# HKUST-Aerial-Robotics/A-LOAM

Hardware: AMD Instinct MI355X
Metric: HDL-64 scans/sec (whole node) (higher is better)
Workload: dtype f32 features / f64 solve

## Files before the change

### a-loam_amd/csrc/odometry_kernels.hip

```cpp
#include "aloam_device.hpp"
#include "aloam_trig.hpp"
#include "lm_device.hpp"
#include "odometry_solve_device.hpp"
#include "odometry_kernels.hpp"

namespace aloam {

#define ALOAM_PHASE(name) asm volatile("; ##PHASE " name)
#ifdef ALOAM_PHASE_CLOCK
__device__ unsigned long long g_phase_clock_odo[2][32];
#define ALOAM_BG_CLOCK(slot) do { if (threadIdx.x == 0 && blockIdx.x == 1) { atomicAdd(&g_phase_clock_odo[0][slot], (unsigned long long)__builtin_readcyclecounter()); atomicAdd(&g_phase_clock_odo[1][slot], 1ull); } } while (0)
#else
#define ALOAM_BG_CLOCK(slot) do { } while (0)
#endif
#ifdef ALOAM_ASSOC_STATS
__device__ unsigned long long g_assoc_stats[2][32];
#define ALOAM_STAT(cls, i, v) do { if ((threadIdx.x & 63) == 0) atomicAdd(&g_assoc_stats[cls][i], (unsigned long long)(v)); } while (0)
#else
#define ALOAM_STAT(cls, i, v) do { } while (0)
#endif

__device__ __forceinline__ float4 transform_to_start(const float4& p, const OdomState& st) {
  double q[4] = {st.para_q[0], st.para_q[1], st.para_q[2], st.para_q[3]};
  if (q[3] < 0.0) { q[0] = -q[0]; q[1] = -q[1]; q[2] = -q[2]; q[3] = -q[3]; }
  double o[3];
  quat_rotate(q, (double)p.x, (double)p.y, (double)p.z, o);
  return make_float4((float)(o[0] + st.para_t[0]), (float)(o[1] + st.para_t[1]), (float)(o[2] + st.para_t[2]), p.w);
}

constexpr float kCell3Surf = 0.5f;
constexpr float kCell3Corner = 0.75f;
constexpr float kCell3CoarseFactor = 4.0f, kCell2 = 2.625f;
constexpr unsigned kIdxMask = (1u << 20) - 1u;
__device__ __forceinline__ float cell3_of(int which) { return which == 0 ? kCell3Corner : kCell3Surf; }

__device__ __forceinline__ unsigned hash3(int a, int b, int c) {
  return ((unsigned)a * 73856093u) ^ ((unsigned)b * 19349663u) ^ ((unsigned)c * 83492791u);
}

constexpr int kFusedMaxN = 65535, kFusedMaxH = 16384;
constexpr int kWalkKeys = kMaxRings + 8;

__device__ __forceinline__ void walk_tables(const float4* __restrict__ pts, int n, int R, int* __restrict__ walk, int* s_walk, int* s_flag, int tid) {
  const int S = R + 8, lane = tid & 63;
  int* s_first = s_walk;
  int* s_last = s_walk + kWalkKeys;
  for (int k = tid; k < kWalkKeys; k += 1024) { s_first[k] = 0x7fffffff; s_last[k] = -1; }
  __syncthreads();
  for (int base = 0; base < n; base += 1024) {
    const int i = base + tid;
    const int key = i < n ? (int)pts[i].w : -1;
    const int prev = __shfl_up(key, 1, 64), next = __shfl_down(key, 1, 64);
    if (key >= 0 && key < S) {
      if (lane == 0 || prev != key) atomicMin(&s_first[key], i);
      if (lane == 63 || next != key) atomicMax(&s_last[key], i);
    }
  }
  __syncthreads();
  if (tid == 0) {
    int run = n;
    for (int k = S - 1; k >= 0; --k) { run = min(run, s_first[k]); s_first[k] = run; walk[k] = run; }
    run = -1;
    for (int k = 0; k < S; ++k) { run = max(run, s_last[k]); s_last[k] = run; walk[S + k] = run; }
    bool nearly = true;
    for (int k = 3; k < S; ++k) nearly = nearly && s_last[k - 3] < s_first[k];
    s_flag[1] = nearly ? 1 : 2;
  }
  __syncthreads();
}
__host__ __device__ __forceinline__ bool fused_takes(int n, int H) { return n <= kFusedMaxN && H <= kFusedMaxH; }

template <bool NEXT>
struct BuildSrc {
  int n, set;
  const float4* pts;
  __device__ __forceinline__ BuildSrc(const OdomArgs& a, const SeqMeta& m, int b, int which) {
    set = NEXT ? m.parity : m.parity ^ 1;
    n = which == 0 ? (NEXT ? m.n_less_sharp : m.n_corner_last) : (NEXT ? m.n_less_flat : m.n_surf_last);
    pts = which == 0 ? row_of(a.less_sharp, set, b, (long long)a.R * kLessSharpPerRing) : row_of(a.less_flat, set, b, (long long)a.cap);
  }
};

template <bool NEXT>
__device__ __forceinline__ void build_grids_fused(const OdomArgs& a, int b, int which) {
  constexpr int U = 4;
  const int tid = threadIdx.x, lane = tid & 63, wave = tid >> 6;
  if (seq_idle(a.active, b, NEXT ? kSeqActive : kSeqSolve)) return;
  const SeqMeta m = a.meta[b];
  const BuildSrc<NEXT> src(a, m, b, which);
  const int n = src.n;
  const float4* pts = src.pts;
  const GridView g = grid_view(a, b, which, src.set);
  const int H = g.H;
  if (!fused_takes(n, H)) return;
  extern __shared__ __attribute__((aligned(16))) int lds[];
  unsigned* tab = reinterpret_cast<unsigned*>(lds);
  int* s_part = lds + 3 * (H / 2);
  int* s_flag = s_part + 48;
  int* s_walk = s_flag + 8;
  int* const starts[3] = {g.start3, g.start3c, g.start2};
  if (n == 0) {
    for (int t = 0; t < 3; ++t) for (int h = tid; h <= H; h += 1024) starts[t][h] = 0;
    if (tid < 3) g.flags[tid] = 0;
    return;
  }
  ALOAM_BG_CLOCK(0);
  for (int w = tid; w < 3 * (H / 2); w += 1024) tab[w] = 0u;
  if (tid < 2) s_flag[tid] = 0;
  __syncthreads();
  ALOAM_BG_CLOCK(1);
  const float inv0 = 1.0f / cell3_of(which), inv1 = 1.0f / (cell3_of(which) * kCell3CoarseFactor), inv2 = 1.0f / kCell2;
  const unsigned hm = (unsigned)(H - 1);
  auto buckets = [&](const float4& p, int key, unsigned* h) {
    h[0] = hash3((int)floorf(p.x * inv0), (int)floorf(p.y * inv0), (int)floorf(p.z * inv0)) & hm;
    h[1] = hash3((int)floorf(p.x * inv1), (int)floorf(p.y * inv1), (int)floorf(p.z * inv1)) & hm;
    h[2] = hash3((int)floorf(p.x * inv2), (int)floorf(p.y * inv2), key) & hm;
  };
  auto fetch = [&](int base, float4* p) {
#pragma unroll
    for (int u = 0; u < U; ++u) { const int i = base + u * 1024 + tid; p[u] = pts[i < n ? i : n - 1]; }
  };
  {
    int bad = 0, unsorted = 0;
    for (int base = 0; base < n; base += U * 1024) {
      float4 p[U];
      float pw[U];
      fetch(base, p);
#pragma unroll
      for (int u = 0; u < U; ++u) { const int i = base + u * 1024 + tid; pw[u] = pts[i < n ? (i > 0 ? i - 1 : 0) : n - 1].w; }
#pragma unroll
      for (int u = 0; u < U; ++u) {
        if (base + u * 1024 + tid >= n) continue;
        const int key = (int)p[u].w;
        if (key < 0 || key > a.R || !(fabsf(p[u].x) < 4096.f && fabsf(p[u].y) < 4096.f && fabsf(p[u].z) < 4096.f)) bad = 1;
        if (key < (int)pw[u]) unsorted = 1;
        unsigned h[3];
        buckets(p[u], key, h);
#pragma unroll
        for (int t = 0; t < 3; ++t) atomicAdd(&tab[t * (H / 2) + (h[t] >> 1)], 1u << ((h[t] & 1u) * 16));
      }
    }
    if (bad) atomicOr(&s_flag[0], 1);
    if (unsorted) atomicOr(&s_flag[1], 1);
  }
  __syncthreads();
  ALOAM_BG_CLOCK(2);
  if (s_flag[1] && !s_flag[0]) walk_tables(pts, n, a.R, g.walk, s_walk, s_flag, tid);
  if (tid < 3) g.flags[tid] = tid == 2 ? 0 : s_flag[tid];
  ALOAM_BG_CLOCK(3);
  {
    const int wpt = H / 2048;
    int local[3], inc[3];
#pragma unroll
    for (int t = 0; t < 3; ++t) {
      local[t] = 0;
      for (int k = 0; k < wpt; ++k) { const unsigned w = tab[t * (H / 2) + tid * wpt + k]; local[t] += (int)(w & 0xffffu) + (int)(w >> 16); }
      inc[t] = wave_scan_i32<false>(local[t]);
      if (lane == 63) s_part[t * 16 + wave] = inc[t];
    }
    __syncthreads();
#pragma unroll
    for (int t = 0; t < 3; ++t) {
      int run = inc[t] - local[t];
#pragma unroll 1
      for (int w = 0; w < wave; ++w) run += s_part[t * 16 + w];
      int* st = starts[t] + tid * wpt * 2;
      for (int k = 0; k < wpt; ++k) {
        const unsigned w = tab[t * (H / 2) + tid * wpt + k];
        const int c0 = (int)(w & 0xffffu), c1 = (int)(w >> 16);
        st[2 * k] = run; st[2 * k + 1] = run + c0;
        tab[t * (H / 2) + tid * wpt + k] = (unsigned)run | ((unsigned)(run + c0) << 16);
        run += c0 + c1;
      }
      if (tid == 1023) starts[t][H] = run;
    }
  }
  __syncthreads();
  ALOAM_BG_CLOCK(4);
  for (int base = 0; base < n; base += U * 1024) {
    float4 p[U];
    fetch(base, p);
#pragma unroll
    for (int u = 0; u < U; ++u) {
      const int i = base + u * 1024 + tid;
      if (i >= n) continue;
      const int key = (int)p[u].w;
      unsigned h[3];
      buckets(p[u], key, h);
      unsigned pos[3];
#pragma unroll
      for (int t = 0; t < 3; ++t) {
        const unsigned sh = (h[t] & 1u) * 16;
        pos[t] = (atomicAdd(&tab[t * (H / 2) + (h[t] >> 1)], 1u << sh) >> sh) & 0xffffu;
      }
      const float4 e = make_float4(p[u].x, p[u].y, p[u].z, __uint_as_float((unsigned)i | ((unsigned)(key + 1) << 20)));
      g.sorted3[pos[0]] = e;
      g.sorted3c[pos[1]] = e;
      g.sorted2[pos[2]] = e;
    }
  }
  ALOAM_BG_CLOCK(5);
#ifdef ALOAM_PHASE_CLOCK
  __syncthreads();
  ALOAM_BG_CLOCK(6);
#endif
}

__global__ __launch_bounds__(1024) void k_build_grids_fused(OdomArgs a) { build_grids_fused<false>(a, blockIdx.y, blockIdx.x); }
__global__ __launch_bounds__(1024) void k_build_grids_fused_next(OdomArgs a) {
  const int G = gridDim.x;
  for (int r = 0, i = blockIdx.x; i < 2 * a.B; ++r, i += G) {
    build_grids_fused<true>(a, i >> 1, (i ^ r) & 1);
    __syncthreads();
  }
}

constexpr int kBgWaves = 4;
constexpr int kBgUnroll = 4;
template <bool NEXT>
__device__ __forceinline__ void build_grids(const OdomArgs& a) {
  constexpr int U = kBgUnroll;
  const int b = blockIdx.y, which = blockIdx.x / 3, tid = threadIdx.x;
  const int pass_lo = blockIdx.x % 3, pass_hi = pass_lo + 1;
  if (seq_idle(a.active, b, NEXT ? kSeqActive : kSeqSolve)) return;
  const SeqMeta m = a.meta[b];
  const BuildSrc<NEXT> src(a, m, b, which);
  const int n = src.n;
  const float4* pts = src.pts;
  const GridView g = grid_view(a, b, which, src.set);
  if (fused_takes(n, g.H)) return;
  extern __shared__ __attribute__((aligned(16))) int lds[];
  int* cnt = lds;
  int* part = lds + g.H;
  int* s_flag = part + 1024;
  if (tid < 2) s_flag[tid] = n >= (1 << 20) && tid == 0 ? 1 : 0;
  if (n == 0) {
    for (int pass = pass_lo; pass < pass_hi; ++pass) { int* st = pass == 0 ? g.start3 : pass == 1 ? g.start3c : g.start2; for (int h = tid; h <= g.H; h += 1024) st[h] = 0; }
    if (tid < 3 && pass_lo == 0) g.flags[tid] = 0;
    return;
  }
  auto fetch = [&](int base, float4* p) {
#pragma unroll
    for (int u = 0; u < U; ++u) { const int i = base + u * 1024 + tid; p[u] = pts[i < n ? i : n - 1]; }
  };
  for (int pass = pass_lo; pass < pass_hi; ++pass) {
    const bool g3 = pass < 2;
    const float cell = pass == 0 ? cell3_of(which) : pass == 1 ? cell3_of(which) * kCell3CoarseFactor : kCell2;
    const float inv = 1.0f / cell;
    int* start = pass == 0 ? g.start3 : pass == 1 ? g.start3c : g.start2;
    float4* sorted = pass == 0 ? g.sorted3 : pass == 1 ? g.sorted3c : g.sorted2;
    __syncthreads();
    for (int h = tid; h < g.H; h += 1024) cnt[h] = 0;
    __syncthreads();
    float4 p[U], pn[U];
    float pw[U], pwn[U];
    fetch(0, p);
    if (pass == 0) {
#pragma unroll
      for (int u = 0; u < U; ++u) { const int i = u * 1024 + tid; pw[u] = pts[i < n ? (i > 0 ? i - 1 : 0) : n - 1].w; }
    }
    int bad = 0, unsorted = 0;
    for (int base = 0; base < n; base += U * 1024) {
      if (base + U * 1024 < n) {
        fetch(base + U * 1024, pn);
        if (pass == 0) {
#pragma unroll
          for (int u = 0; u < U; ++u) { const int i = base + U * 1024 + u * 1024 + tid; pwn[u] = pts[i < n ? i - 1 : n - 1].w; }
        }
      }
#pragma unroll
      for (int u = 0; u < U; ++u) {
        if (base + u * 1024 + tid >= n) continue;
        const int key = (int)p[u].w;
        if (pass == 0) {
          if (key < 0 || key > a.R || !(fabsf(p[u].x) < 4096.f && fabsf(p[u].y) < 4096.f && fabsf(p[u].z) < 4096.f)) bad = 1;
          if (key < (int)pw[u]) unsorted = 1;
        }
        const int ix = (int)floorf(p[u].x * inv), iy = (int)floorf(p[u].y * inv);
        const int iz = g3 ? (int)floorf(p[u].z * inv) : key;
        atomicAdd(&cnt[hash3(ix, iy, iz) & (g.H - 1)], 1);
      }
#pragma unroll
      for (int u = 0; u < U; ++u) { p[u] = pn[u]; pw[u] = pwn[u]; }
    }
    if (pass == 0) {
      if (bad) atomicOr(&s_flag[0], 1);
      if (unsorted) atomicOr(&s_flag[1], 1);
    }
    __syncthreads();
    if (pass == 0 && tid < 3) g.flags[tid] = tid == 2 ? 0 : (tid == 1 ? 2 * s_flag[1] : s_flag[0]);
    const int per = g.H / 1024;
    int local = 0;
    for (int k = 0; k < per; ++k) local += cnt[tid * per + k];
    int total;
    int run = block_exclusive_scan<int, 1024>(local, part, &total);
    for (int k = 0; k < per; ++k) { const int c = cnt[tid * per + k]; cnt[tid * per + k] = run; start[tid * per + k] = run; run += c; }
    if (tid == 1023) start[g.H] = run;
    __syncthreads();
    fetch(0, p);
    for (int base = 0; base < n; base += U * 1024) {
      if (base + U * 1024 < n) fetch(base + U * 1024, pn);
#pragma unroll
      for (int u = 0; u < U; ++u) {
        const int i = base + u * 1024 + tid;
        if (i >= n) continue;
        const int key = (int)p[u].w;
        const int ix = (int)floorf(p[u].x * inv), iy = (int)floorf(p[u].y * inv);
        const int iz = g3 ? (int)floorf(p[u].z * inv) : key;
        const int pos = atomicAdd(&cnt[hash3(ix, iy, iz) & (g.H - 1)], 1);
        sorted[pos] = make_float4(p[u].x, p[u].y, p[u].z, __uint_as_float((unsigned)i | ((unsigned)(key + 1) << 20)));
      }
#pragma unroll
      for (int u = 0; u < U; ++u) p[u] = pn[u];
    }
  }
}

__global__ __launch_bounds__(1024, kBgWaves) void k_build_grids(OdomArgs a) { build_grids<false>(a); }
__global__ __launch_bounds__(1024, kBgWaves) void k_build_grids_next(OdomArgs a) { build_grids<true>(a); }

__device__ __forceinline__ float walk_dist(const float4& p, const float4& sel) {
  return (p.x - sel.x) * (p.x - sel.x) + (p.y - sel.y) * (p.y - sel.y) + (p.z - sel.z) * (p.z - sel.z);
}

__device__ __forceinline__ unsigned long long wave_min_u64(unsigned long long v) {
  return wave_min_packed(v);
}

__device__ __forceinline__ void ring2d(int r, int t, int* dx, int* dy) {
  const int w = 2 * r + 1;
  if (t < w) { *dx = -r + t; *dy = -r; }
  else if (t < 2 * w) { *dx = -r + (t - w); *dy = r; }
  else { const int u = t - 2 * w, side = u / (w - 2); *dy = -r + 1 + u % (w - 2); *dx = side ? r : -r; }
}
__device__ __forceinline__ void shell3d(int r, int c, int* dx, int* dy, int* dz) {
  const int w = 2 * r + 1, nface = w * w;
  if (c < 2 * nface) { const int f = c / nface, q = c % nface; *dz = f ? r : -r; *dy = q / w - r; *dx = q % w - r; }
  else { const int q = c - 2 * nface; *dz = -r + 1 + q / (8 * r); ring2d(r, q % (8 * r), dx, dy); }
}

template <int kSweep> struct Kept { float4 p[kSweep]; bool a[kSweep]; bool ok; };

template <int kSweep, class F>
__device__ __forceinline__ void wave_sweep(const float4* __restrict__ sorted, int s0, int cnt, int lane, int* row, F&& f, Kept<kSweep>* keep = nullptr) {
  const int incl = wave_scan_i32<false>(cnt);
  const int total = __builtin_amdgcn_readlane(incl, 63);
  const int excl = incl - cnt;
  int carry = 0;
  for (int base = 0; base < total; base += kSweep * 64) {
    const int slot = excl - base;
    const int rows = total - base > (kSweep - 1) * 64 ? kSweep : (total - base + 63) >> 6;
#pragma unroll
    for (int u = 0; u < kSweep; ++u) if (u < rows) row[u * 64 + lane] = 0;
    __builtin_amdgcn_wave_barrier();
    if (cnt > 0 && slot >= 0 && slot < rows * 64) row[slot] = lane + 1;
    __builtin_amdgcn_wave_barrier();
    int own[kSweep];
#pragma unroll
    for (int u = 0; u < kSweep; ++u) own[u] = u < rows ? row[u * 64 + lane] : 0;
    __builtin_amdgcn_wave_barrier();
    float4 p[kSweep];
#pragma unroll
    for (int u = 0; u < kSweep; ++u) {
      p[u] = make_float4(0.f, 0.f, 0.f, 0.f);
      if (u < rows) {
        if (lane == 0 && carry > own[u]) own[u] = carry;
        own[u] = wave_scan_i32<true>(own[u]);
        carry = __builtin_amdgcn_readlane(own[u], 63);
        const int i = base + u * 64 + lane;
        const int os = __shfl(s0, own[u] - 1, 64), oe = __shfl(excl, own[u] - 1, 64);
        const int at = i < total ? os + (i - oe) : 0;
        p[u] = sorted[at];
      }
    }
#pragma unroll
    for (int u = 0; u < kSweep; ++u) {
      const bool act = u < rows && base + u * 64 + lane < total;
      if (keep) { keep->p[u] = p[u]; keep->a[u] = act; }
      if (act) f(p[u]);
    }
  }
  if (keep) keep->ok = total <= kSweep * 64;
}

__device__ __forceinline__ float cell_gap(float s, int c, float cell) {
  const float lo = (float)c * cell, hi = lo + cell;
  const float gap = s < lo ? lo - s : (s > hi ? s - hi : 0.f);
  return gap > 1e-3f ? gap - 1e-3f : 0.f;
}

struct Track { unsigned long long v; float x, y, z; };
__device__ __forceinline__ void track_take(Track& t, bool ok, unsigned long long v, const float4& p) {
  const bool k = ok && v < t.v;
  t.v = k ? v : t.v; t.x = k ? p.x : t.x; t.y = k ? p.y : t.y; t.z = k ? p.z : t.z;
}

template <int kSweep>
__device__ __forceinline__ unsigned long long wave_nn(const GridView& g, bool bad, int which, const float4* pts, int n, const float4& sel, int lane, int* row, Track& mine, Kept<kSweep>& kept) {
  unsigned long long best = ~0ull;
  auto visit = [&](const float4& p) {
    const float ddx = p.x - sel.x, ddy = p.y - sel.y, ddz = p.z - sel.z;
    const float d = (ddx * ddx + ddy * ddy) + ddz * ddz;
    const unsigned wb = __float_as_uint(p.w);
    track_take(mine, true, ((unsigned long long)__float_as_uint(d) << 32) | ((wb & kIdxMask) << 12) | (wb >> 20), p);
  };
  if (!bad) {
    const float cell = cell3_of(which);
    {
      const float inv = 1.0f / cell;
      const int cx = (int)floorf(sel.x * inv), cy = (int)floorf(sel.y * inv), cz = (int)floorf(sel.z * inv);
      int s0 = 0, cnt = 0;
      if (lane < 27) {
        const unsigned h = hash3(cx + lane % 3 - 1, cy + (lane % 9) / 3 - 1, cz + lane / 9 - 1) & (unsigned)(g.H - 1);
        s0 = g.start3[h];
        cnt = g.start3[h + 1] - s0;
      }
      wave_sweep<kSweep>(g.sorted3, s0, cnt, lane, row, visit, &kept);
      best = wave_min_u64(mine.v);
      const float bound = (1.0f - 0.01f) * cell;
      if (best != ~0ull && __uint_as_float((unsigned)(best >> 32)) <= bound * bound) return best;
    }
    const float cellc = cell * kCell3CoarseFactor, invc = 1.0f / cellc;
    const int ux = (int)floorf(sel.x * invc), uy = (int)floorf(sel.y * invc), uz = (int)floorf(sel.z * invc);
    for (int r = 1;; ++r) {
      const int ncell = r == 1 ? 27 : 24 * r * r + 2;
      const float limit = best != ~0ull ? fminf(__uint_as_float((unsigned)(best >> 32)), 25.0f) : 25.0f;
      for (int cb = 0; cb < ncell; cb += 64) {
        const int c = cb + lane;
        int s0 = 0, cnt = 0;
        if (c < ncell) {
          int dx, dy, dz;
          if (r == 1) { dz = c / 9 - 1; dy = (c % 9) / 3 - 1; dx = c % 3 - 1; }
          else shell3d(r, c, &dx, &dy, &dz);
          const float gx = cell_gap(sel.x, ux + dx, cellc), gy = cell_gap(sel.y, uy + dy, cellc), gz = cell_gap(sel.z, uz + dz, cellc);
          if (((gx * gx + gy * gy) + gz * gz) * 0.999f <= limit) {
            const unsigned h = hash3(ux + dx, uy + dy, uz + dz) & (unsigned)(g.H - 1);
            s0 = g.start3c[h];
            cnt = g.start3c[h + 1] - s0;
          }
        }
        wave_sweep<kSweep>(g.sorted3c, s0, cnt, lane, row, visit);
      }
      best = wave_min_u64(mine.v);
      const float bc = ((float)r - 0.01f) * cellc, b2 = bc * bc;
      if (best != ~0ull && __uint_as_float((unsigned)(best >> 32)) <= b2) break;
      if (b2 >= 25.0f) break;
    }
    return best;
  }
  for (int base = 0; base < n; base += 64) {
    const int j = base + lane;
    if (j < n) {
      const float4 p = pts[j];
      visit(make_float4(p.x, p.y, p.z, __uint_as_float((unsigned)j)));
    }
  }
  return wave_min_u64(mine.v);
}

template <bool DISTORT>
__global__ __launch_bounds__(256) void k_transform_queries(OdomArgs a) {
  const int b = blockIdx.y, i = blockIdx.x * 256 + threadIdx.x;
  if (seq_idle(a.active, b, kSeqSolve)) return;
  const SeqMeta m = a.meta[b];
  if (i >= m.n_sharp + m.n_flat) return;
  const bool plane = i >= m.n_sharp;
  const int qi = plane ? i - m.n_sharp : i;
  const long long o = plane ? (long long)b * a.R * kFlatPerRing + qi : (long long)b * a.R * kSharpPerRing + qi;
  const float4 raw = plane ? a.flat[o] : a.sharp[o];
  float4 sel;
  if (DISTORT) {
    const OdomState& st = a.state[b];
    const double q[4] = {st.para_q[0], st.para_q[1], st.para_q[2], st.para_q[3]}, t[3] = {st.para_t[0], st.para_t[1], st.para_t[2]};
    const float frac = raw.w - (float)(int)raw.w;
    double lp[3];
    deskew_point(q, t, interpolation_ratio(frac), (double)raw.x, (double)raw.y, (double)raw.z, lp, nullptr);
    sel = make_float4((float)lp[0], (float)lp[1], (float)lp[2], raw.w);
  } else sel = transform_to_start(raw, a.state[b]);
  (plane ? a.sel_flat : a.sel_sharp)[o] = sel;
}

constexpr int kAssocSweepWide = 6;
constexpr int kAssocSweepPlane = 3;
template <bool PLANE, bool WIDE> struct SweepRows { static constexpr int value = WIDE ? (PLANE ? kAssocSweepWide : 3) : (PLANE ? kAssocSweepPlane : 2); };

template <bool PLANE, bool WIDE>
__device__ __forceinline__ void associate_one(const OdomArgs& a, int b, int qi, const SeqMeta& m, const GridView& g, int lane, int* row) {
  constexpr int kSweep = SweepRows<PLANE, WIDE>::value;
  const int qcap = PLANE ? a.R * kFlatPerRing : a.R * kSharpPerRing;
  const float4* Q = (PLANE ? a.flat : a.sharp) + (long long)b * qcap;
  const float4 raw = Q[qi];
  const float4 sel = ((PLANE ? a.sel_flat : a.sel_sharp) + (long long)b * qcap)[qi];
  const bool bad = g.flags[0] != 0, unsorted = g.flags[1] != 0;
  const float frac = raw.w - (float)(int)raw.w;
  const int nt = PLANE ? m.n_surf_last : m.n_corner_last;
  const float4* T = PLANE ? surf_last(a, b, m.parity) : corner_last(a, b, m.parity);
  int valid = 0;
  Track t1 = {~0ull, 0.f, 0.f, 0.f}, t2 = t1, t3 = t1;
  Kept<kSweep> kept;
  kept.ok = false;
#pragma unroll
  for (int u = 0; u < kSweep; ++u) { kept.a[u] = false; kept.p[u] = make_float4(0.f, 0.f, 0.f, 0.f); }
  unsigned long long best2 = ~0ull, best3 = ~0ull;
  const unsigned long long nn = nt > 0 ? wave_nn(g, bad, PLANE ? 1 : 0, T, nt, sel, lane, row, t1, kept) : ~0ull;
  const float nnd = __uint_as_float((unsigned)(nn >> 32));
  if (nn != ~0ull && (double)nnd < 25.0) {
    const int closest = (int)((unsigned)nn >> 12);
    const int cid = bad ? (int)T[closest].w : (int)((unsigned)nn & 0xfffu) - 1;
    auto consider = [&](const float4& p, int j, int key) {
      if (j == closest) return;
      const bool up = j > closest;
      bool c2, c3;
      if (PLANE) { c2 = up ? key <= cid : key >= cid; c3 = !c2; }
      else { c2 = up ? key > cid : key < cid; c3 = false; }
      const float d = walk_dist(p, sel);
      if (!((double)d < 25.0)) return;
      const unsigned seq = up ? (unsigned)(j - closest) : 0x40000000u + (unsigned)(closest - j);
      const unsigned long long v = ((unsigned long long)__float_as_uint(d) << 32) | seq;
      track_take(t2, c2, v, p);
      if (PLANE) track_take(t3, c3, v, p);
    };
    if (!bad && !unsorted) {
      auto visit = [&](const float4& p) {
        const unsigned wb = __float_as_uint(p.w);
        const int j = (int)(wb & kIdxMask), pk = (int)(wb >> 20) - 1;
        if (pk >= cid - 2 && pk <= cid + 2) consider(p, j, pk);
      };
      bool done2 = false, done3 = !PLANE;
      float lim2 = 25.0f, lim3 = 25.0f;
      if (kept.ok) {
#pragma unroll
        for (int u = 0; u < kSweep; ++u) if (kept.a[u]) visit(kept.p[u]);
        best2 = wave_min_u64(t2.v);
        if (PLANE) best3 = wave_min_u64(t3.v);
        const float bound = (1.0f - 0.01f) * cell3_of(PLANE ? 1 : 0), b2 = bound * bound;
        if (best2 != ~0ull) lim2 = __uint_as_float((unsigned)(best2 >> 32));
        if (PLANE && best3 != ~0ull) lim3 = __uint_as_float((unsigned)(best3 >> 32));
        done2 = best2 != ~0ull && lim2 <= b2;
        done3 = !PLANE || (best3 != ~0ull && lim3 <= b2);
      }
      for (int level = 0; level < 2 && !(done2 && done3); ++level) {
        const float cell = kCell2, inv = 1.0f / cell;
        const int cx = (int)floorf(sel.x * inv), cy = (int)floorf(sel.y * inv);
        const int nlook = level == 0 ? 45 : 80;
        for (int lb = 0; lb < nlook; lb += 64) {
          const int l = lb + lane;
          int s0 = 0, cnt = 0;
          if (l < nlook) {
            const int key = cid + l % 5 - 2, cc = l / 5;
            int ddx, ddy;
            if (level == 0) { ddx = cc % 3 - 1; ddy = cc / 3 - 1; }
            else ring2d(2, cc, &ddx, &ddy);
            const bool second = PLANE ? key == cid : key != cid;
            const bool wanted = second ? !done2 : (PLANE && !done3);
            const float gx = cell_gap(sel.x, cx + ddx, cell), gy = cell_gap(sel.y, cy + ddy, cell);
            if (key >= 0 && wanted && (gx * gx + gy * gy) * 0.999f <= (second ? lim2 : lim3)) {
              const unsigned h = hash3(cx + ddx, cy + ddy, key) & (unsigned)(g.H - 1);
              s0 = g.start2[h];
              cnt = g.start2[h + 1] - s0;
            }
          }
          wave_sweep<kSweep>(g.sorted2, s0, cnt, lane, row, visit);
        }
        best2 = wave_min_u64(t2.v);
        if (PLANE) best3 = wave_min_u64(t3.v);
        const float bound = ((float)(level + 1) - 0.01f) * cell, b2 = bound * bound;
        if (b2 >= 25.0f) break;
        if (best2 != ~0ull) lim2 = __uint_as_float((unsigned)(best2 >> 32));
        if (PLANE && best3 != ~0ull) lim3 = __uint_as_float((unsigned)(best3 >> 32));
        done2 = best2 != ~0ull && lim2 <= b2;
        done3 = !PLANE || (best3 != ~0ull && lim3 <= b2);
      }
    } else {
      for (int base = closest + 1; base < nt; base += 64) {
        const int j = base + lane;
        bool stop = false;
        float4 p = make_float4(0.f, 0.f, 0.f, 0.f);
        int key = 0;
        if (j < nt) { p = T[j]; key = (int)p.w; stop = (double)key > (double)cid + 2.5; }
        const unsigned long long sm = __ballot(stop);
        const int first_stop = sm ? (__ffsll((long long)sm) - 1) : 64;
        if (j < nt && lane < first_stop) consider(p, j, key);
        if (sm) break;
      }
      for (int base = closest - 1; base >= 0; base -= 64) {
        const int j = base - lane;
        bool stop = false;
        float4 p = make_float4(0.f, 0.f, 0.f, 0.f);
        int key = 0;
        if (j >= 0) { p = T[j]; key = (int)p.w; stop = (double)key < (double)cid - 2.5; }
        const unsigned long long sm = __ballot(stop);
        const int first_stop = sm ? (__ffsll((long long)sm) - 1) : 64;
        if (j >= 0 && lane < first_stop) consider(p, j, key);
        if (sm) break;
      }
      best2 = wave_min_u64(t2.v);
      if (PLANE) best3 = wave_min_u64(t3.v);
    }
    valid = best2 != ~0ull && (!PLANE || best3 != ~0ull);
  }
  if (PLANE) {
    PlaneRec* e = a.planes + (long long)b * a.R * kFlatPerRing + qi;
    if (lane == 0) {
      e->cp[0] = raw.x; e->cp[1] = raw.y; e->cp[2] = raw.z;
      e->valid = valid; e->pad[0] = __float_as_int(frac); e->pad[1] = e->pad[2] = 0;
      if (!valid) for (int k = 0; k < 3; ++k) e->j[k] = e->l[k] = e->m[k] = 0.f;
    }
    if (valid) {
      if (t1.v == nn) { e->j[0] = t1.x; e->j[1] = t1.y; e->j[2] = t1.z; }
      if (t2.v == best2) { e->l[0] = t2.x; e->l[1] = t2.y; e->l[2] = t2.z; }
      if (t3.v == best3) { e->m[0] = t3.x; e->m[1] = t3.y; e->m[2] = t3.z; }
    }
  } else {
    EdgeRec* e = a.edges + (long long)b * a.R * kSharpPerRing + qi;
    if (lane == 0) {
      e->cp[0] = raw.x; e->cp[1] = raw.y; e->cp[2] = raw.z;
      e->valid = valid; e->pad[0] = __float_as_int(frac); e->pad[1] = 0;
      if (!valid) for (int k = 0; k < 3; ++k) e->a[k] = e->b[k] = 0.f;
    }
    if (valid) {
      if (t1.v == nn) { e->a[0] = t1.x; e->a[1] = t1.y; e->a[2] = t1.z; }
      if (t2.v == best2) { e->b[0] = t2.x; e->b[1] = t2.y; e->b[2] = t2.z; }
// ... 240 lines not shown
    for (int lb = 0; lb < n_look; lb += W) {
      const int k = lb + l;
      int s0 = 0, cnt = 0;
      const bool centre = k >= ncell * nslot;
      const int slot = centre ? k - ncell * nslot : k >> lc;
      const bool other = slot < 4;
      if (k < n_look && (other ? wo : ws)) {
        const int key = cid - 2 + (int)((0x2819u >> (slot * 3)) & 7u);
        int ddx = 0, ddy = 0;
        float gx = 0.f, gy = 0.f;
        if (stage > 0 && !centre) {
          const CellOff2 o = kRingCells[(stage == 1 ? 0 : 8) + (k & (ncell - 1))];
          ddx = o.dx; ddy = o.dy;
          gx = axis_gap(ddx, o.ax, ax); gy = axis_gap(ddy, o.ay, ay);
        }
        const bool second = PLANE ? !other : true;
        if (key >= 0 && (gx * gx + gy * gy) * 0.999f <= (second ? lim2 : lim3)) {
          const unsigned hh = hash3(cx + ddx, cy + ddy, key) & hm;
          bucket_bounds(g.start2, hh, s0, cnt);
        }
      }
      ALOAM_PHASE("ring_sweep");
      sweep2<HALVES, kRows>(g.sorted2, last_index, s0, cnt, lane, last4, lds, [&](const float4& p, int, bool) {
        const unsigned wb = __float_as_uint(p.w);
        consider2<PLANE, NEARLY>(dist_to(p, sxy, sz), (int)(wb & kIdxMask), (int)(wb >> 20) - 1, closest, cid, t2, t3, lo, hi);
      }, nullptr, nullptr, PLANE ? 1 : 0, 8 + 4 * stage);
    }
    ALOAM_PHASE("ring_mins");
    if (!PLANE || track2) best2 = seg_min<HALVES>(t2, last4);
    if (PLANE) best3 = seg_min<HALVES>(t3, last4);
    ALOAM_PHASE("ring_bounds");
    if (stage == 2) break;
    float bound;
    if (stage == 0) bound = (1.0f - 0.01f) * fmaxf(fminf(fminf(ax.up, ax.dn), fminf(ay.up, ay.dn)) + rc, 0.f);
    else bound = ((float)stage - 0.01f) * rc;
    const float b2 = bound * bound;
    if (!none(best2)) lim2 = __uint_as_float((unsigned)(best2 >> 32));
    if (PLANE && !none(best3)) lim3 = __uint_as_float((unsigned)(best3 >> 32));
    if (!none(best2) && lim2 <= b2) want2 = false;
    if (PLANE && !none(best3) && lim3 <= b2) want3 = false;
  }
}

__device__ __forceinline__ unsigned long long read_u64(unsigned long long v, int src) {
  return ((unsigned long long)(unsigned)__builtin_amdgcn_readlane((int)(unsigned)(v >> 32), src) << 32) | (unsigned)__builtin_amdgcn_readlane((int)(unsigned)v, src);
}
__device__ __forceinline__ float read_f32(float v, int src) { return __int_as_float(__builtin_amdgcn_readlane(__float_as_int(v), src)); }

template <bool PLANE, int kRows, bool PAIRED_TAILS, bool NEARLY>
__device__ __forceinline__ void associate_pair(const OdomArgs& a, int b, int qi0, int nq, int nt, const GridView& g, int lane, int* lds) {
  constexpr int kRows1 = (kRows + 1) / 2;
  const int l = lane & 31, hsel = lane >> 5, last4 = (lane | 31) << 2;
  const int qi = qi0 + hsel;
  const bool qact = qi < nq;
  const int qcap = PLANE ? a.R * kFlatPerRing : a.R * kSharpPerRing;
  const long long qo = (long long)b * qcap + (qact ? qi : qi0);
  const float4 raw = (PLANE ? a.flat : a.sharp)[qo];
  const float4 sel = (PLANE ? a.sel_flat : a.sel_sharp)[qo];
  const float frac = raw.w - (float)(int)raw.w;
  const int parity = a.meta[b].parity;
  const float4* T = PLANE ? surf_last(a, b, parity) : corner_last(a, b, parity);
  const unsigned hm = (unsigned)(g.H - 1), last_index = (unsigned)(nt - 1);
  const float cell = cell3_of(PLANE ? 1 : 0);
  const float2v selxy = {sel.x, sel.y};

  ALOAM_PHASE("setup");
  unsigned long long t1 = ~0ull;
  KeptPair<kRows> kept;
  int kept_rows = 0;
#pragma unroll
  for (int u = 0; u < kRows; ++u) kept.k[u] = ~0ull;
  {
    const float inv = 1.0f / cell;
    const int cx = (int)floorf(sel.x * inv), cy = (int)floorf(sel.y * inv), cz = (int)floorf(sel.z * inv);
    int s0 = 0, cnt = 0;
    if (l < 27 && qact) {
      const unsigned hh = hash3(cx + l % 3 - 1, cy + (l % 9) / 3 - 1, cz + l / 9 - 1) & hm;
      bucket_bounds(g.start3, hh, s0, cnt);
    }
    sweep2<true, kRows>(g.sorted3, last_index, s0, cnt, lane, last4, lds, [&](const float4& p, int u, bool first) {
      const unsigned long long v = nn_key(dist_to(p, selxy, sel.z), __float_as_uint(p.w));
      if (first) kept.k[u] = v;
      take_min(t1, v);
    }, &kept.ok, &kept_rows, PLANE ? 1 : 0, 4);
  }
  ALOAM_PHASE("nn_min");
  unsigned long long nn = half_min_packed(t1, last4);
  float fine_b2;
  {
    const float inv = 1.0f / cell;
    const float lx = floorf(sel.x * inv) * cell, ly = floorf(sel.y * inv) * cell, lz = floorf(sel.z * inv) * cell;
    const float gap = fminf(fminf(fminf(sel.x - lx, (lx + cell) - sel.x), fminf(sel.y - ly, (ly + cell) - sel.y)), fminf(sel.z - lz, (lz + cell) - sel.z));
    const float b = (1.0f - 0.01f) * (cell + (gap > 1e-3f ? gap - 1e-3f : 0.f));
    fine_b2 = b * b;
  }
  {
    const float bound2 = fine_b2;
    const bool need1 = qact && !(nn != ~0ull && __uint_as_float((unsigned)(nn >> 32)) <= bound2);
    const unsigned long long need = __ballot(need1);
    const bool n0 = need & 1ull, n1 = (need >> 32) & 1ull;
    if (PAIRED_TAILS && n0 && n1) nn = coarse_shells<kRows1, true>(g, last_index, cell * kCell3CoarseFactor, sel.x, sel.y, sel.z, nn, need1, lane, last4, lds, PLANE ? 1 : 0);
    else if (n0 || n1) {
      const int q = n0 ? 0 : 1;
#pragma unroll
      for (int qq = 0; qq < 2; ++qq) {
        if (PAIRED_TAILS ? qq != q : !((need >> (32 * qq)) & 1ull)) continue;
        const unsigned long long r = coarse_shells<kRows1, false>(g, last_index, cell * kCell3CoarseFactor, read_f32(sel.x, 32 * qq), read_f32(sel.y, 32 * qq), read_f32(sel.z, 32 * qq),
                                                                    read_u64(nn, 32 * qq), true, lane, 0, lds, PLANE ? 1 : 0);
        if (hsel == qq) nn = r;
      }
    }
  }
  ALOAM_PHASE("classes");
  const float nnd = __uint_as_float((unsigned)(nn >> 32));
  const bool has1 = qact && nn != ~0ull && nnd < 25.0f;
  const int closest = (int)((unsigned)nn >> 12);
  const int cid = (int)((unsigned)nn & 0xfffu) - 1;
  unsigned long long best2 = ~0ull, best3 = ~0ull;
  int wlo = -1, whi = nt;
  if (NEARLY && has1) {
    const int S = a.R + 8, c = min(max(cid, 0), a.R);
    whi = g.walk[c + 3];
    wlo = c >= 3 ? g.walk[S + c - 3] : -1;
  }
  ALOAM_STAT(PLANE ? 1 : 0, 0, 1); ALOAM_STAT(PLANE ? 1 : 0, 1, (int)((__ballot(qact) & 1) + ((__ballot(qact) >> 32) & 1))); ALOAM_STAT(PLANE ? 1 : 0, 2, (int)((__ballot(has1) & 1) + ((__ballot(has1) >> 32) & 1)));
  ALOAM_STAT(PLANE ? 1 : 0, 3, (int)((__ballot(has1 && kept.ok) & 1) + ((__ballot(has1 && kept.ok) >> 32) & 1)));
  if (__ballot(has1)) {
    bool want2 = has1, want3 = PLANE && has1;
    if (__ballot(has1 && kept.ok)) {
      unsigned long long t2 = ~0ull, t3 = ~0ull;
#pragma unroll
      for (int u = 0; u < kRows; ++u) {
        if (u >= kept_rows) continue;
        const unsigned lo = (unsigned)kept.k[u];
        consider2<PLANE, NEARLY>(__uint_as_float((unsigned)(kept.k[u] >> 32)), (int)(lo >> 12), (int)(lo & 0xfffu) - 1, closest, cid, t2, t3, wlo, whi);
      }
      const bool use = has1 && kept.ok;
      best2 = half_min_packed(use ? t2 : ~0ull, last4);
      if (PLANE) best3 = half_min_packed(use ? t3 : ~0ull, last4);
      const float b2 = fine_b2;
      if (!none(best2) && __uint_as_float((unsigned)(best2 >> 32)) <= b2) want2 = false;
      if (PLANE && !none(best3) && __uint_as_float((unsigned)(best3 >> 32)) <= b2) want3 = false;
    }
    ALOAM_PHASE("ring_tail");
    const unsigned long long w2 = __ballot(want2), w3 = __ballot(want3);
    const bool r0 = (w2 | w3) & 1ull, r1 = ((w2 | w3) >> 32) & 1ull;
    if (PAIRED_TAILS && r0 && r1) ring_grid<PLANE, kRows1, true, NEARLY>(g, last_index, sel.x, sel.y, sel.z, closest, cid, want2, want3, best2, best3, lane, last4, lds, wlo, whi);
    else {
#pragma unroll
      for (int q = 0; q < 2; ++q) {
        const bool q2 = (w2 >> (32 * q)) & 1ull, q3 = (w3 >> (32 * q)) & 1ull;
        if (!(q2 || q3)) continue;
        unsigned long long r2 = read_u64(best2, 32 * q), r3 = read_u64(best3, 32 * q);
        ring_grid<PLANE, kRows1, false, NEARLY>(g, last_index, read_f32(sel.x, 32 * q), read_f32(sel.y, 32 * q), read_f32(sel.z, 32 * q), __builtin_amdgcn_readlane(closest, 32 * q),
                                                __builtin_amdgcn_readlane(cid, 32 * q), q2, q3, r2, r3, lane, 0, lds, __builtin_amdgcn_readlane(wlo, 32 * q), __builtin_amdgcn_readlane(whi, 32 * q));
        if (hsel == q) { best2 = r2; best3 = r3; }
      }
    }
  }
  ALOAM_PHASE("record");
  const bool valid = has1 && !none(best2) && (!PLANE || !none(best3));

  if (qact) {
    constexpr int kPts = PLANE ? 4 : 3;
    float* e = PLANE ? reinterpret_cast<float*>(a.planes + (long long)b * a.R * kFlatPerRing + qi) : reinterpret_cast<float*>(a.edges + (long long)b * a.R * kSharpPerRing + qi);
    if (l < kPts) {
      float x = raw.x, y = raw.y, z = raw.z;
      if (l > 0) {
        x = y = z = 0.f;
        if (valid) {
          const int j = l == 1 ? closest : index_of(l == 2 ? best2 : best3, closest);
          const float4 p = T[j];
          x = p.x; y = p.y; z = p.z;
        }
      }
      e[3 * l] = x; e[3 * l + 1] = y; e[3 * l + 2] = z;
    } else if (l == kPts) {
      int* ei = reinterpret_cast<int*>(e) + 3 * kPts;
      ei[0] = valid ? 1 : 0; ei[1] = __float_as_int(frac); ei[2] = 0;
      if (PLANE) ei[3] = 0;
    }
  }
}

template <bool PLANE, bool WIDE>
__global__ __launch_bounds__(64) void k_associate_pair(OdomArgs a) {
  constexpr int kRows = PairRows<PLANE, WIDE>::value;
  __shared__ int lds[sweep2_lds_ints<kRows>()];
  const int lane = threadIdx.x, L = blockIdx.x, xcd = L & 7, slot = L >> 3;
  const int pairs = PLANE ? a.R * (kFlatPerRing / 2) : a.R * (kSharpPerRing / 2);
  const int b = (slot / pairs) * 8 + xcd, qi0 = (slot % pairs) * 2;
  if (b >= a.B || seq_idle(a.active, b, kSeqSolve)) return;
  const SeqMeta m = a.meta[b];
  const int nq = PLANE ? m.n_flat : m.n_sharp;
  if (qi0 >= nq) return;
  const GridView g = grid_view(a, b, PLANE ? 1 : 0, m.parity ^ 1);
  const int nt = PLANE ? m.n_surf_last : m.n_corner_last;
  if (g.flags[0] != 0 || g.flags[1] != 0 || nt <= 0) return;
  associate_pair<PLANE, kRows, !WIDE, false>(a, b, qi0, nq, nt, g, lane, lds);
}

constexpr int kPairsPerWave = 8;
template <bool PLANE, bool WIDE>
__global__ __launch_bounds__(64) void k_associate_nearly(OdomArgs a) {
  constexpr int kRows = PairRows<PLANE, WIDE>::value;
  __shared__ int lds[sweep2_lds_ints<kRows>()];
  const int lane = threadIdx.x, b = blockIdx.y;
  if (seq_idle(a.active, b, kSeqSolve)) return;
  const SeqMeta m = a.meta[b];
  const GridView g = grid_view(a, b, PLANE ? 1 : 0, m.parity ^ 1);
  if (g.flags[0] != 0 || g.flags[1] != 1) return;
  const int nq = PLANE ? m.n_flat : m.n_sharp, nt = PLANE ? m.n_surf_last : m.n_corner_last;
  if (nt <= 0) return;
  for (int k = 0; k < kPairsPerWave; ++k) {
    const int qi0 = (blockIdx.x * kPairsPerWave + k) * 2;
    if (qi0 >= nq) return;
    associate_pair<PLANE, kRows, !WIDE, true>(a, b, qi0, nq, nt, g, lane, lds);
  }
}

template <bool PLANE, bool WIDE>
__global__ __launch_bounds__(256) void k_associate_flagged(OdomArgs a) {
  constexpr int kSweep = SweepRows<PLANE, WIDE>::value;
  __shared__ int rows[4][kSweep * 64];
  const int b = blockIdx.x, lane = threadIdx.x & 63, wave = threadIdx.x >> 6;
  if (seq_idle(a.active, b, kSeqSolve)) return;
  const SeqMeta m = a.meta[b];
  const GridView g = grid_view(a, b, PLANE ? 1 : 0, m.parity ^ 1);
  const int nt = PLANE ? m.n_surf_last : m.n_corner_last;
  if (!(g.flags[0] != 0 || g.flags[1] == 2 || nt <= 0)) return;
  const int nq = PLANE ? m.n_flat : m.n_sharp;
  for (int qi = wave; qi < nq; qi += 4) associate_one<PLANE, WIDE>(a, b, qi, m, g, lane, rows[wave]);
}

template <bool DISTORT>
__global__ __launch_bounds__(kSolveThreads) void k_solve(OdomArgs a) {
  const int b = blockIdx.x, tid = threadIdx.x;
  __shared__ double s_red[kSolveWaves * 28];
  if (seq_idle(a.active, b, kSeqSolve)) return;
  OdomState& st = a.state[b];
  double q[4] = {st.para_q[0], st.para_q[1], st.para_q[2], st.para_q[3]};
  double t[3] = {st.para_t[0], st.para_t[1], st.para_t[2]};

  const LmResult lm = lm_solve_block<kSolveWaves>([&](bool with_jac, const double* qq, const double* tt, double* acc, int* ne, int* np) {
    if (with_jac) evaluate<true, DISTORT>(a, b, qq, tt, acc, ne, np); else evaluate<false, DISTORT>(a, b, qq, tt, acc, ne, np);
  }, q, t, a.lm_max_iterations, s_red);
  const int n_edges = lm.n_a, n_planes = lm.n_b, iterations = lm.iterations, successful = lm.successful, termination = lm.termination;
  const double initial_cost = lm.initial_cost, cost = lm.final_cost;

  if (tid == 0) {
    if (termination == 5) {
      for (int k = 0; k < 4; ++k) q[k] = st.para_q[k];
      for (int k = 0; k < 3; ++k) t[k] = st.para_t[k];
    }
    for (int k = 0; k < 4; ++k) st.para_q[k] = q[k];
    for (int k = 0; k < 3; ++k) st.para_t[k] = t[k];
    const int o = a.outer < 2 ? a.outer : 1;
    st.corner_corr[o] = n_edges;
    st.plane_corr[o] = n_planes;
    st.lm_iterations[o] = iterations;
    st.lm_successful[o] = successful;
    st.initial_cost[o] = initial_cost;
    st.final_cost[o] = cost;
    st.termination[o] = termination;
    if (a.last_outer) {
      const double qw[4] = {st.q_w[0], st.q_w[1], st.q_w[2], st.q_w[3]};
      double rt[3];
      quat_rotate(qw, t[0], t[1], t[2], rt);
      st.t_w[0] += rt[0]; st.t_w[1] += rt[1]; st.t_w[2] += rt[2];
      st.q_w[0] = qw[3] * q[0] + qw[0] * q[3] + qw[1] * q[2] - qw[2] * q[1];
      st.q_w[1] = qw[3] * q[1] + qw[1] * q[3] + qw[2] * q[0] - qw[0] * q[2];
      st.q_w[2] = qw[3] * q[2] + qw[2] * q[3] + qw[0] * q[1] - qw[1] * q[0];
      st.q_w[3] = qw[3] * q[3] - qw[0] * q[0] - qw[1] * q[1] - qw[2] * q[2];
    }
  }
}

__global__ void k_advance(SeqMeta* meta, OdomState* state, const int* active, int B) {
  const int b = blockIdx.x * blockDim.x + threadIdx.x;
  if (b >= B || seq_idle(active, b)) return;
  SeqMeta& m = meta[b];
  m.n_corner_last = m.n_less_sharp; m.n_surf_last = m.n_less_flat; m.parity ^= 1;
  state[b].inited = 1;
}
__global__ void k_set_inited(OdomState* state, int B, int inited) {
  const int b = blockIdx.x * blockDim.x + threadIdx.x;
  if (b < B) state[b].inited = inited;
}
void launch_set_inited(OdomState* state, int B, int inited, hipStream_t s) { hipLaunchKernelGGL(k_set_inited, dim3((B + 63) / 64), dim3(64), 0, s, state, B, inited); }
void launch_advance(const OdomArgs& a, hipStream_t s) { hipLaunchKernelGGL(k_advance, dim3((a.B + 63) / 64), dim3(64), 0, s, a.meta, a.state, a.active, a.B); }

size_t build_grids_lds_bytes(int H, int R) { return sizeof(int) * ((size_t)H + 1024 + 2 * (R + 8) + 4); }
static size_t build_grids_fused_lds_bytes(int H) { return sizeof(int) * (3 * (size_t)(H / 2) + 48 + 8 + 2 * kWalkKeys); }
int prepare_build_grids(int H_surf) {
  const int fused = (int)build_grids_fused_lds_bytes(kFusedMaxH), per_grid = (int)build_grids_lds_bytes(H_surf, kMaxRings);
  if (hipFuncSetAttribute((const void*)k_build_grids_fused, hipFuncAttributeMaxDynamicSharedMemorySize, fused) != hipSuccess) return -1;
  if (hipFuncSetAttribute((const void*)k_build_grids_fused_next, hipFuncAttributeMaxDynamicSharedMemorySize, fused) != hipSuccess) return -1;
  if (hipFuncSetAttribute((const void*)k_build_grids, hipFuncAttributeMaxDynamicSharedMemorySize, per_grid) != hipSuccess) return -1;
  return hipFuncSetAttribute((const void*)k_build_grids_next, hipFuncAttributeMaxDynamicSharedMemorySize, per_grid) == hipSuccess ? 0 : -1;
}
void launch_build_grids(const OdomArgs& a, bool next, int cus, hipStream_t s) {
  const int hc = a.grid_H_corner <= kFusedMaxH ? a.grid_H_corner : 0, hs = a.grid_H_surf <= kFusedMaxH ? a.grid_H_surf : 0;
  const size_t fused = build_grids_fused_lds_bytes(hc > hs ? hc : hs), per_grid = build_grids_lds_bytes(a.grid_H_surf, a.R);
  if (next) {
    const int wgs = cus / 2 >= 2 ? (cus / 2) & ~1 : 2;
    if (hc || hs) hipLaunchKernelGGL(k_build_grids_fused_next, dim3(2 * a.B < wgs ? 2 * a.B : wgs), dim3(1024), fused, s, a);
    hipLaunchKernelGGL(k_build_grids_next, dim3(6, a.B), dim3(1024), per_grid, s, a);
  } else {
    if (hc || hs) hipLaunchKernelGGL(k_build_grids_fused, dim3(2, a.B), dim3(1024), fused, s, a);
    hipLaunchKernelGGL(k_build_grids, dim3(6, a.B), dim3(1024), per_grid, s, a);
  }
}
void launch_transform_queries(const OdomArgs& a, hipStream_t s) {
  const dim3 grid((a.R * (kSharpPerRing + kFlatPerRing) + 255) / 256, a.B);
  if (a.distortion) hipLaunchKernelGGL(k_transform_queries<true>, grid, dim3(256), 0, s, a);
  else hipLaunchKernelGGL(k_transform_queries<false>, grid, dim3(256), 0, s, a);
}
void launch_associate(const OdomArgs& a, bool plane, hipStream_t s) {
  const int by = (a.B + 7) / 8 * 8;
  const int qcap = plane ? a.R * kFlatPerRing : a.R * kSharpPerRing;
  const bool wide = a.R > 64;
  const dim3 grid((unsigned)(qcap / 2 * by)), block(64), gridf((unsigned)a.B), blockf(256);
  const dim3 gridn((unsigned)((qcap / 2 + kPairsPerWave - 1) / kPairsPerWave), (unsigned)a.B);
  if (wide) {
    if (plane) { hipLaunchKernelGGL((k_associate_pair<true, true>), grid, block, 0, s, a); hipLaunchKernelGGL((k_associate_nearly<true, true>), gridn, block, 0, s, a); hipLaunchKernelGGL((k_associate_flagged<true, true>), gridf, blockf, 0, s, a); }
    else { hipLaunchKernelGGL((k_associate_pair<false, true>), grid, block, 0, s, a); hipLaunchKernelGGL((k_associate_nearly<false, true>), gridn, block, 0, s, a); hipLaunchKernelGGL((k_associate_flagged<false, true>), gridf, blockf, 0, s, a); }
  } else {
    if (plane) { hipLaunchKernelGGL((k_associate_pair<true, false>), grid, block, 0, s, a); hipLaunchKernelGGL((k_associate_nearly<true, false>), gridn, block, 0, s, a); hipLaunchKernelGGL((k_associate_flagged<true, false>), gridf, blockf, 0, s, a); }
    else { hipLaunchKernelGGL((k_associate_pair<false, false>), grid, block, 0, s, a); hipLaunchKernelGGL((k_associate_nearly<false, false>), gridn, block, 0, s, a); hipLaunchKernelGGL((k_associate_flagged<false, false>), gridf, blockf, 0, s, a); }
  }
}
void launch_solve(const OdomArgs& a, hipStream_t s) {
  if (a.distortion) hipLaunchKernelGGL(k_solve<true>, dim3(a.B), dim3(kSolveThreads), 0, s, a);
  else hipLaunchKernelGGL(k_solve<false>, dim3(a.B), dim3(kSolveThreads), 0, s, a);
}
}

#ifdef ALOAM_PHASE_CLOCK
extern "C" int aloam_debug_phase_clock_odo(unsigned long long* out) { return (int)hipMemcpyFromSymbol(out, HIP_SYMBOL(aloam::g_phase_clock_odo), sizeof(unsigned long long) * 64); }
#endif
#ifdef ALOAM_ASSOC_STATS
extern "C" int aloam_debug_assoc_stats(unsigned long long* out) { return (int)hipMemcpyFromSymbol(out, HIP_SYMBOL(aloam::g_assoc_stats), sizeof(unsigned long long) * 64); }
#endif
```

Before: 135,500.

## Double-buffer fused grid-build loads and skip corner fallback blocks

The fused grid build now uses a two-group software pipeline, so the next chunk of points is fetched while the current chunk is hashed and counted or scattered. The per-point previous-key global reload is replaced by a DPP lane shift, with only lane 0 loading the neighbour. The unroll depth differs between the last-frame and next-frame kernels. The fallback per-grid build kernel no longer launches the three corner blocks when the fused path handles corners, which cuts idle workgroups. Together these add register pressure and code complexity, and the DPP row-shift semantics must hold across wave rows.

```diff
diff --git a/a-loam_amd/csrc/odometry_kernels.hip b/a-loam_amd/csrc/odometry_kernels.hip
--- a/a-loam_amd/csrc/odometry_kernels.hip
+++ b/a-loam_amd/csrc/odometry_kernels.hip
@@ -81,9 +81,47 @@
   }
 };
 
-template <bool NEXT>
+#ifndef ALOAM_BG_NEXT_U
+#define ALOAM_BG_NEXT_U 4
+#endif
+constexpr int kFusedPtsLast = 2, kFusedPtsNext = ALOAM_BG_NEXT_U;
+
+template <int U, bool PREV>
+struct FusedGroup {
+  float4 p[U];
+  float pw[PREV ? U : 1];
+  __device__ __forceinline__ void landed() {
+#pragma unroll
+    for (int u = 0; u < U; ++u) asm volatile("" : "+v"(p[u].x), "+v"(p[u].y), "+v"(p[u].z), "+v"(p[u].w));
+#pragma unroll
+    for (int u = 0; u < (PREV ? U : 0); ++u) asm volatile("" : "+v"(pw[u]));
+  }
+};
+template <class G, class Fetch, class Full, class Ragged>
+__device__ __forceinline__ void fused_rounds(int n, int GP, Fetch fetch, Full full, Ragged ragged) {
+  G g0, g1;
+  fetch(0, g0);
+  g0.landed();
+  int base = 0;
+  bool odd = false;
+  while (base + GP <= n) {
+    fetch(base + GP, g1);
+    full(g0, base);
+    base += GP;
+    if (base + GP > n) { odd = true; break; }
+    fetch(base + GP, g0);
+    full(g1, base);
+    base += GP;
+  }
+  if (base < n) {
+    if (odd) g0 = g1;
+    ragged(g0, base);
+  }
+}
+
+template <bool NEXT, int U>
 __device__ __forceinline__ void build_grids_fused(const OdomArgs& a, int b, int which) {
-  constexpr int U = 4;
+  constexpr int GP = U * 1024;
   const int tid = threadIdx.x, lane = tid & 63, wave = tid >> 6;
   if (seq_idle(a.active, b, NEXT ? kSeqActive : kSeqSolve)) return;
   const SeqMeta m = a.meta[b];
@@ -116,30 +154,35 @@
     h[1] = hash3((int)floorf(p.x * inv1), (int)floorf(p.y * inv1), (int)floorf(p.z * inv1)) & hm;
     h[2] = hash3((int)floorf(p.x * inv2), (int)floorf(p.y * inv2), key) & hm;
   };
-  auto fetch = [&](int base, float4* p) {
-#pragma unroll
-    for (int u = 0; u < U; ++u) { const int i = base + u * 1024 + tid; p[u] = pts[i < n ? i : n - 1]; }
-  };
   {
+    using Grp = FusedGroup<U, true>;
+    auto fetch = [&](int base, Grp& q) {
+#pragma unroll
+      for (int u = 0; u < U; ++u) { const int i = base + u * 1024 + tid; q.p[u] = pts[i < n ? i : n - 1]; }
+#pragma unroll
+      for (int u = 0; u < U; ++u) { const int i = base + u * 1024 + tid; q.pw[u] = 0.f; if (lane == 0) q.pw[u] = pts[i < n ? (i > 0 ? i - 1 : 0) : n - 1].w; }
+    };
     int bad = 0, unsorted = 0;
-    for (int base = 0; base < n; base += U * 1024) {
-      float4 p[U];
-      float pw[U];
-      fetch(base, p);
-#pragma unroll
-      for (int u = 0; u < U; ++u) { const int i = base + u * 1024 + tid; pw[u] = pts[i < n ? (i > 0 ? i - 1 : 0) : n - 1].w; }
-#pragma unroll
-      for (int u = 0; u < U; ++u) {
-        if (base + u * 1024 + tid >= n) continue;
-        const int key = (int)p[u].w;
-        if (key < 0 || key > a.R || !(fabsf(p[u].x) < 4096.f && fabsf(p[u].y) < 4096.f && fabsf(p[u].z) < 4096.f)) bad = 1;
-        if (key < (int)pw[u]) unsorted = 1;
-        unsigned h[3];
-        buckets(p[u], key, h);
-#pragma unroll
-        for (int t = 0; t < 3; ++t) atomicAdd(&tab[t * (H / 2) + (h[t] >> 1)], 1u << ((h[t] & 1u) * 16));
-      }
-    }
+    auto count = [&](const float4& p, float pw, bool live) {
+      const int key = (int)p.w;
+      const int prev = __builtin_amdgcn_update_dpp((int)pw, key, 0x138, 0xF, 0xF, false);
+      if (!live) return;
+      bad |= (key < 0 || key > a.R || !(fabsf(p.x) < 4096.f && fabsf(p.y) < 4096.f && fabsf(p.z) < 4096.f)) ? 1 : 0;
+      unsorted |= key < prev ? 1 : 0;
+      unsigned h[3];
+      buckets(p, key, h);
+#pragma unroll
+      for (int t = 0; t < 3; ++t) atomicAdd(&tab[t * (H / 2) + (h[t] >> 1)], 1u << ((h[t] & 1u) * 16));
+    };
+    fused_rounds<Grp>(n, GP, fetch,
+      [&](const Grp& q, int) {
+#pragma unroll
+        for (int u = 0; u < U; ++u) count(q.p[u], q.pw[u], true);
+      },
+      [&](const Grp& q, int base) {
+#pragma unroll
+        for (int u = 0; u < U; ++u) count(q.p[u], q.pw[u], base + u * 1024 + tid < n);
+      });
     if (bad) atomicOr(&s_flag[0], 1);
     if (unsorted) atomicOr(&s_flag[1], 1);
   }
@@ -177,27 +220,36 @@
   }
   __syncthreads();
   ALOAM_BG_CLOCK(4);
-  for (int base = 0; base < n; base += U * 1024) {
-    float4 p[U];
-    fetch(base, p);
-#pragma unroll
-    for (int u = 0; u < U; ++u) {
-      const int i = base + u * 1024 + tid;
-      if (i >= n) continue;
-      const int key = (int)p[u].w;
+  {
+    auto place = [&](const float4& p, int i) {
+      const int key = (int)p.w;
       unsigned h[3];
-      buckets(p[u], key, h);
+      buckets(p, key, h);
       unsigned pos[3];
 #pragma unroll
       for (int t = 0; t < 3; ++t) {
         const unsigned sh = (h[t] & 1u) * 16;
         pos[t] = (atomicAdd(&tab[t * (H / 2) + (h[t] >> 1)], 1u << sh) >> sh) & 0xffffu;
       }
-      const float4 e = make_float4(p[u].x, p[u].y, p[u].z, __uint_as_float((unsigned)i | ((unsigned)(key + 1) << 20)));
+      const float4 e = make_float4(p.x, p.y, p.z, __uint_as_float((unsigned)i | ((unsigned)(key + 1) << 20)));
       g.sorted3[pos[0]] = e;
       g.sorted3c[pos[1]] = e;
       g.sorted2[pos[2]] = e;
-    }
+    };
+    using Grp = FusedGroup<U, false>;
+    fused_rounds<Grp>(n, GP,
+      [&](int base, Grp& q) {
+#pragma unroll
+        for (int u = 0; u < U; ++u) { const int i = base + u * 1024 + tid; q.p[u] = pts[i < n ? i : n - 1]; }
+      },
+      [&](const Grp& q, int base) {
+#pragma unroll
+        for (int u = 0; u < U; ++u) place(q.p[u], base + u * 1024 + tid);
+      },
+      [&](const Grp& q, int base) {
+#pragma unroll
+        for (int u = 0; u < U; ++u) { const int i = base + u * 1024 + tid; if (i < n) place(q.p[u], i); }
+      });
   }
   ALOAM_BG_CLOCK(5);
 #ifdef ALOAM_PHASE_CLOCK
@@ -206,11 +258,11 @@
 #endif
 }
 
-__global__ __launch_bounds__(1024) void k_build_grids_fused(OdomArgs a) { build_grids_fused<false>(a, blockIdx.y, blockIdx.x); }
+__global__ __launch_bounds__(1024) void k_build_grids_fused(OdomArgs a) { build_grids_fused<false, kFusedPtsLast>(a, blockIdx.y, blockIdx.x); }
 __global__ __launch_bounds__(1024) void k_build_grids_fused_next(OdomArgs a) {
   const int G = gridDim.x;
   for (int r = 0, i = blockIdx.x; i < 2 * a.B; ++r, i += G) {
-    build_grids_fused<true>(a, i >> 1, (i ^ r) & 1);
+    build_grids_fused<true, kFusedPtsNext>(a, i >> 1, (i ^ r) & 1);
     __syncthreads();
   }
 }
@@ -218,10 +270,10 @@
 constexpr int kBgWaves = 4;
 constexpr int kBgUnroll = 4;
 template <bool NEXT>
-__device__ __forceinline__ void build_grids(const OdomArgs& a) {
+__device__ __forceinline__ void build_grids(const OdomArgs& a, int first) {
   constexpr int U = kBgUnroll;
-  const int b = blockIdx.y, which = blockIdx.x / 3, tid = threadIdx.x;
-  const int pass_lo = blockIdx.x % 3, pass_hi = pass_lo + 1;
+  const int b = blockIdx.y, which = (blockIdx.x + first) / 3, tid = threadIdx.x;
+  const int pass_lo = (blockIdx.x + first) % 3, pass_hi = pass_lo + 1;
   if (seq_idle(a.active, b, NEXT ? kSeqActive : kSeqSolve)) return;
   const SeqMeta m = a.meta[b];
   const BuildSrc<NEXT> src(a, m, b, which);
@@ -316,8 +368,8 @@
   }
 }
 
-__global__ __launch_bounds__(1024, kBgWaves) void k_build_grids(OdomArgs a) { build_grids<false>(a); }
-__global__ __launch_bounds__(1024, kBgWaves) void k_build_grids_next(OdomArgs a) { build_grids<true>(a); }
+__global__ __launch_bounds__(1024, kBgWaves) void k_build_grids(OdomArgs a, int first) { build_grids<false>(a, first); }
+__global__ __launch_bounds__(1024, kBgWaves) void k_build_grids_next(OdomArgs a, int first) { build_grids<true>(a, first); }
 
 __device__ __forceinline__ float walk_dist(const float4& p, const float4& sel) {
   return (p.x - sel.x) * (p.x - sel.x) + (p.y - sel.y) * (p.y - sel.y) + (p.z - sel.z) * (p.z - sel.z);
@@ -1164,13 +1216,19 @@
 void launch_build_grids(const OdomArgs& a, bool next, int cus, hipStream_t s) {
   const int hc = a.grid_H_corner <= kFusedMaxH ? a.grid_H_corner : 0, hs = a.grid_H_surf <= kFusedMaxH ? a.grid_H_surf : 0;
   const size_t fused = build_grids_fused_lds_bytes(hc > hs ? hc : hs), per_grid = build_grids_lds_bytes(a.grid_H_surf, a.R);
+  static_assert(kMaxRings * kLessSharpPerRing <= kFusedMaxN, "a corner cloud the fused build cannot take");
+  const int first = hc ? 3 : 0;
   if (next) {
+#ifdef ALOAM_BG_NEXT_WGS
+    const int wgs = ALOAM_BG_NEXT_WGS;
+#else
     const int wgs = cus / 2 >= 2 ? (cus / 2) & ~1 : 2;
+#endif
     if (hc || hs) hipLaunchKernelGGL(k_build_grids_fused_next, dim3(2 * a.B < wgs ? 2 * a.B : wgs), dim3(1024), fused, s, a);
-    hipLaunchKernelGGL(k_build_grids_next, dim3(6, a.B), dim3(1024), per_grid, s, a);
+    hipLaunchKernelGGL(k_build_grids_next, dim3(6 - first, a.B), dim3(1024), per_grid, s, a, first);
   } else {
     if (hc || hs) hipLaunchKernelGGL(k_build_grids_fused, dim3(2, a.B), dim3(1024), fused, s, a);
-    hipLaunchKernelGGL(k_build_grids, dim3(6, a.B), dim3(1024), per_grid, s, a);
+    hipLaunchKernelGGL(k_build_grids, dim3(6 - first, a.B), dim3(1024), per_grid, s, a, first);
   }
 }
 void launch_transform_queries(const OdomArgs& a, hipStream_t s) {
```

Measured after the change: 133,800. 1.2% lower.
